# scenarios/VAE-2

Measured on AMD Instinct MI355X. Metric: training frames/sec on 128x256 8-frame Cityscapes clips, 1/2/4/8 MI355X, higher is better.
Workload: dtype fp32; 1 GPU; VAE2 ELBO step (encz + encoder + 2 decoders fwd/bwd + Adam), HRNet-W18-small-v2, 128x256, 8 clips/GPU x 9 frames (CLIP_LENGTH=3); yaml=vae-2_amd/experiments/vae2_w18_small_v2_128x256.yaml, global_batch=8, frames_per_clip=9, parallelism=dp1, sync_bn=False, launch=hip_graph, mfma_operands=fp32

## Files before the change

### vae-2_amd/csrc/common.h

```cpp
#pragma once

#include <hip/hip_runtime.h>
#include <stdint.h>
#include <string>
#include <stdio.h>

#include "../../include/vae2_hip.h"

namespace vae2 {

constexpr int kSyncMaxRanks = 8;

void set_error(const std::string& msg);
int fail(const char* fn, const std::string& msg);
int check_launch(const char* fn);

void note_kernel(const void* host_fn);
#define VAE2_LAUNCH(K, ...)                                         \
  do {                                                              \
    ::vae2::note_kernel(reinterpret_cast<const void*>(K));          \
    hipLaunchKernelGGL(K, __VA_ARGS__);                             \
  } while (0)

#define VAE2_REQUIRE(cond, fn, msg)          \
// ... 123 lines not shown
struct FastDiv {
  uint32_t d, m, s;
  FastDiv() : d(1), m(0), s(0) {}
  explicit FastDiv(uint32_t div) : d(div) {
    for (s = 0; s < 32; ++s)
      if ((1u << s) >= d) break;
    uint64_t one = 1;
    m = (uint32_t)(((one << 32) * ((one << s) - d)) / d + 1);
  }
  __device__ __forceinline__ uint32_t div(uint32_t n) const {
    return (__umulhi(n, m) + n) >> s;
  }
};

struct Lerp {
  int i0, i1;
  float l0, l1;
};

__device__ __forceinline__ Lerp lerp_index(int dst, int in_size, float scale) {
  float src = scale * ((float)dst + 0.5f) - 0.5f;
  if (src < 0.f) src = 0.f;
  int i0 = (int)src;
  if (i0 > in_size - 1) i0 = in_size - 1;
  int ip = (i0 < in_size - 1) ? 1 : 0;
  Lerp l;
  l.i0 = i0;
  l.i1 = i0 + ip;
  l.l1 = src - (float)i0;
  l.l0 = 1.f - l.l1;
  return l;
}

__device__ __forceinline__ float lerp_weight(int o, int in_size, float scale, int i) {
  Lerp l = lerp_index(o, in_size, scale);
  float w = 0.f;
  if (l.i0 == i) w += l.l0;
  if (l.i1 == i) w += l.l1;
  return w;
}

__device__ constexpr float hat_w(int d, int f) {
  return 1.f - (float)(2 * d + 1 - f < 0 ? f - 1 - 2 * d : 2 * d + 1 - f) / (float)(2 * f);
}

int adj3_fuse_launch(const float* dy, const vae2_act* dyd, int n, float* const* dxs,
                     const vae2_act* dxds, const float* betas, hipStream_t st);
extern int g_relu_dual_q;

int64_t wgrad3n_splits(const vae2_act* xd, const vae2_act* dyd);
int wgrad3n_launch(const float* x, const vae2_act* xd, const float* dy, const vae2_act* dyd,
                   float* part, const float* isave, int irelu, uint32_t x_bytes,
                   uint32_t dy_bytes, hipStream_t s);

extern int g_dconv_stream, g_dconv_stream_wpc, g_dconv_stream_bl, g_dconv_stream_spb,
    g_wgrad_narrow_tps, g_bn_blocks, g_bn_apply_res, g_fuse_quad;
bool dconv3s_shape(const vae2_act* ad, const vae2_act* yd);
int64_t dconv3s_rows(const vae2_act* ad, const vae2_act* yd);
int dconv3s_launch(const float* a, const vae2_act* ad, const float* wp, uint32_t w_bytes,
                   const float* bias, float* y, const vae2_act* yd, float beta, float* stats,
                   bool flip, const float* isave, int irelu, const float* bx, int bx_ps,
                   int brelu, const float* bsave, uint32_t bx_bytes, uint32_t a_bytes,
                   hipStream_t s);

int bias_grad_from_partials(const float* partials, int64_t rows, int64_t c,
                            float* dbias, int accumulate, void* stream);

inline unsigned ew_blocks(int64_t n, int threads = 256, int64_t cap = 65536) {
  int64_t b = ceil_div(n, threads);
  if (b > cap) b = cap;
  if (b < 1) b = 1;
  return (unsigned)b;
}

}
```

### vae-2_amd/csrc/conv.hip

```cpp
#include <mutex>
#include <vector>

#include "common.h"

#ifndef VAE2_ABLATE
#define VAE2_ABLATE 0
#endif

#ifndef VAE2_CONV_PART
#define VAE2_CONV_PART -1
#endif
#define VAE2_PART(n) (VAE2_CONV_PART < 0 || VAE2_CONV_PART == (n))

namespace vae2 {


static inline int round_up(int a, int b) { return (a + b - 1) / b * b; }

#if VAE2_PART(0)
__global__ void pack_weight_kernel(const float* __restrict__ w, int cout, int cin, int kk,
                                   int mode, int ld, float* __restrict__ out) {
  const int rows = mode == 0 ? (cout + 63) / 64 * 64 : (cin + 63) / 64 * 64;
  const int cols4 = mode == 0 ? (cin + 3) / 4 * 4 : (cout + 3) / 4 * 4;
  const int total = rows * kk * cols4;
// ... 575 lines not shown
template <int TM, int TN>
__global__ __launch_bounds__(256) void gemm1x1_kernel(Gemm1 p) {
  constexpr int BN = 16 * TN;
  extern __shared__ __attribute__((aligned(16))) float bsh[];
  __shared__ float red[4][2][BN];
  const int lane = threadIdx.x & 63, wave = threadIdx.x >> 6;
  const int g = lane >> 4, r = lane & 15;
  const int n0 = blockIdx.y * BN;
  const int nch = (p.a_c4 + 15) >> 4;
  const int KL = nch * 16 + 4;
  {
    const __amdgpu_buffer_rsrc_t wr = make_rsrc(p.w, p.w_bytes);
    const int q4 = nch * 4;
    for (int i = threadIdx.x; i < BN * q4; i += 256) {
      const int nn = i / q4, q = i - nn * q4;
      const bool ok = 4 * q < p.a_c4;
      const f4 v = load4(wr, ok ? (uint32_t)((n0 + nn) * p.a_c4 + 4 * q) * 4u : kOOB);
      *reinterpret_cast<f4*>(&bsh[nn * KL + 4 * q]) = v;
    }
  }
  const __amdgpu_buffer_rsrc_t ar = make_rsrc(p.a, p.a_bytes);
  const int ntiles = (p.M + 16 * TM - 1) / (16 * TM);
  const int t0 = blockIdx.x * 4 + wave, tstep = gridDim.x * 4;
  const int iters = t0 < ntiles ? (ntiles - t0 + tstep - 1) / tstep : 0;
  const int S = iters * nch;
  const bool cpad = (p.a_c & 3) != 0;
  float bv[TN];
#pragma unroll
  for (int j = 0; j < TN; ++j) {
    const int n = n0 + j * 16 + r;
    bv[j] = (p.bias && n < p.n) ? p.bias[n] : 0.f;
  }
  f4 acc[TM][TN];
#pragma unroll
  for (int i = 0; i < TM; ++i)
#pragma unroll
    for (int j = 0; j < TN; ++j) acc[i][j] = f4{0.f, 0.f, 0.f, 0.f};
  float csum[TN], csq[TN];
#pragma unroll
  for (int j = 0; j < TN; ++j) { csum[j] = 0.f; csq[j] = 0.f; }
  const bool bnp = p.bx != nullptr;
  float pmn[TN], pis[TN], psc[TN], psh[TN];
#pragma unroll
  for (int j = 0; j < TN; ++j) {
    const int n = n0 + j * 16 + r < p.n ? n0 + j * 16 + r : p.n - 1;
    pmn[j] = bnp ? p.bsave[n] : 0.f;
    pis[j] = bnp ? p.bsave[p.n + n] : 0.f;
    psc[j] = bnp ? p.bsave[2 * p.n + n] : 0.f;
    psh[j] = bnp ? p.bsave[3 * p.n + n] : 0.f;
  }
  const __amdgpu_buffer_rsrc_t bxr = make_rsrc(p.bx, bnp ? p.bx_bytes : 0u);
  __syncthreads();

  auto load = [&](f4* fa, int st) {
    const int it = st / nch, c = st - it * nch;
    const int t = t0 + it * tstep;
    const int q = 16 * c + 4 * g;
#pragma unroll
    for (int i = 0; i < TM; ++i) {
      const int m = t * 16 * TM + i * 16 + r;
      const bool ok = st < S && m < p.M && q < p.a_c4;
      fa[i] = load4(ar, ok ? (uint32_t)(m * p.a_ps + q) * 4u : kOOB);
    }
  };
  auto mma = [&](f4* fa, int st) {
    const int it = st / nch, c = st - it * nch;
    if (cpad && c == nch - 1) {
      const int q = 16 * c + 4 * g;
#pragma unroll
      for (int i = 0; i < TM; ++i) {
        fa[i][1] = q + 1 < p.a_c ? fa[i][1] : 0.f;
        fa[i][2] = q + 2 < p.a_c ? fa[i][2] : 0.f;
        fa[i][3] = q + 3 < p.a_c ? fa[i][3] : 0.f;
      }
    }
    f4 fb[TN];
#pragma unroll
    for (int j = 0; j < TN; ++j)
      fb[j] = *reinterpret_cast<const f4*>(&bsh[(j * 16 + r) * KL + 16 * c + 4 * g]);
#pragma unroll
    for (int s2 = 0; s2 < 4; ++s2)
#pragma unroll
      for (int i = 0; i < TM; ++i)
#pragma unroll
        for (int j = 0; j < TN; ++j)
          acc[i][j] = __builtin_amdgcn_mfma_f32_16x16x4f32(fa[i][s2], fb[j][s2], acc[i][j], 0, 0, 0);
  };
  auto epi = [&](int st) {
    const int it = st / nch, c = st - it * nch;
    if (c != nch - 1) return;
    const int t = t0 + it * tstep;
    const int k = r & 3, qc = 4 * (r >> 2);
#pragma unroll
    for (int i = 0; i < TM; ++i) {
      const int mb = t * 16 * TM + i * 16 + 4 * g;
      if (p.stats && bnp) {
        float xv[4][TN];
#pragma unroll
        for (int e = 0; e < 4; ++e)
#pragma unroll
          for (int j = 0; j < TN; ++j) {
            const int n = n0 + j * 16 + r;
            xv[e][j] = load1(bxr, mb + e < p.M && n < p.n
                                      ? (uint32_t)((mb + e) * p.bx_ps + n) * 4u : kOOB);
          }
#pragma unroll
        for (int e = 0; e < 4; ++e) {
#pragma unroll
          for (int j = 0; j < TN; ++j) {
            const bool ok = mb + e < p.M && n0 + j * 16 + r < p.n;
            const float v = acc[i][j][e];
            const float x = xv[e][j];
            const float gv = (p.brelu && !(__builtin_fmaf(x, psc[j], psh[j]) > 0.f)) ? 0.f : v;
            csum[j] += ok ? gv : 0.f;
            csq[j] += ok ? gv * (x - pmn[j]) * pis[j] : 0.f;
          }
        }
      } else if (p.stats) {
#pragma unroll
        for (int e = 0; e < 4; ++e) {
#pragma unroll
          for (int j = 0; j < TN; ++j) {
            if (mb + e < p.M && n0 + j * 16 + r < p.n) {
              const float v = acc[i][j][e] + bv[j];
              csum[j] += v;
              csq[j] += v * v;
            }
          }
        }
      }
      const int m = mb + k;
      float* yrow = p.y + (int64_t)m * p.y_ps;
      f4 yold[TN];
      if (p.beta != 0.f) {
#pragma unroll
        for (int j = 0; j < TN; ++j) {
          const int n = n0 + j * 16 + qc;
          yold[j] = (p.vec && m < p.M && n + 3 < p.n) ? *reinterpret_cast<const f4*>(yrow + n)
                                                      : f4{0.f, 0.f, 0.f, 0.f};
        }
      }
#pragma unroll
      for (int j = 0; j < TN; ++j) {
        f4 v = acc[i][j];
        acc[i][j] = f4{0.f, 0.f, 0.f, 0.f};
        quad_transpose(v, k);
        const int n = n0 + j * 16 + qc;
        if (m >= p.M || n >= p.n) continue;
        if (p.bias) {
#pragma unroll
          for (int q = 0; q < 4; ++q) v[q] += n + q < p.n ? p.bias[n + q] : 0.f;
        }
        if (p.vec && n + 3 < p.n) {
          if (p.beta != 0.f) v += p.beta * yold[j];
          *reinterpret_cast<f4*>(yrow + n) = v;
        } else {
#pragma unroll
          for (int q = 0; q < 4; ++q)
            if (n + q < p.n) yrow[n + q] = p.beta != 0.f ? v[q] + p.beta * yrow[n + q] : v[q];
        }
      }
    }
  };
  if (S > 0) {
    f4 fa0[TM], fa1[TM];
    load(fa0, 0);
    load(fa1, 1);
    for (int st = 0; st < S; st += 2) {
      mma(fa0, st);
      load(fa0, st + 2);
      epi(st);
      if (st + 1 < S) {
        mma(fa1, st + 1);
        load(fa1, st + 3);
        epi(st + 1);
      }
    }
  }
  if (p.stats) {
#pragma unroll
    for (int j = 0; j < TN; ++j) {
      csum[j] += __shfl_xor(csum[j], 16, 64);
      csum[j] += __shfl_xor(csum[j], 32, 64);
      csq[j] += __shfl_xor(csq[j], 16, 64);
      csq[j] += __shfl_xor(csq[j], 32, 64);
    }
    if (g == 0) {
#pragma unroll
      for (int j = 0; j < TN; ++j) {
        red[wave][0][j * 16 + r] = csum[j];
        red[wave][1][j * 16 + r] = csq[j];
      }
    }
    __syncthreads();
    const int rows = gridDim.x;
    for (int c = threadIdx.x; c < BN; c += 256) {
      if (n0 + c >= p.n) continue;
      p.stats[blockIdx.x * p.n + n0 + c] = red[0][0][c] + red[1][0][c] + red[2][0][c] + red[3][0][c];
      p.stats[(rows + blockIdx.x) * p.n + n0 + c] =
          red[0][1][c] + red[1][1][c] + red[2][1][c] + red[3][1][c];
    }
  }
}

struct DConv {
  const float* a;
  int a_ps, a_c, a_c4, img_h, img_w;
  int tiles_h, tiles_w;
  int cs4;
  const float* w;
  uint32_t a_bytes, w_bytes;
  int n;
  const float* bias;
  float* y;
  int y_ps;
  float beta;
  float* stats;
  const float* isave;
  int irelu;
  const float* bx;
  int bx_ps, brelu;
  const float* bsave;
  uint32_t bx_bytes;
  int vec_out;
};

constexpr int kDcBW = 32;
constexpr int kDcMaxCs4 = 8;
// ... 1858 lines not shown
  }
  if (key == 1) {
    const int prev = g_wgrad_cols;
    g_wgrad_cols = value ? 1 : 0;
    return prev;
  }
  if (key == 2) {
    const int prev = g_dconv_nw8;
    g_dconv_nw8 = value ? 1 : 0;
    return prev;
  }
  if (key == 3) {
    const int prev = g_wgrad_nw8;
    g_wgrad_nw8 = value ? 1 : 0;
    return prev;
  }
  if (key == 4) {
    if (value < 3 || value > 8) return -1;
    const int prev = g_gemm1_tn;
    g_gemm1_tn = value;
    return prev;
  }
  if (key == 5) {
    const int prev = g_gemm1_tm;
    g_gemm1_tm = value == 1 ? 1 : 2;
    return prev;
  }
  if (key == 6) {
    if (value < 0 || value > 2) return -1;
    const int prev = g_igemm_nr;
    g_igemm_nr = value;
    return prev;
  }
  if (key == 8) {
    const int prev = g_bn_v2;
    g_bn_v2 = value ? 1 : 0;
    return prev;
  }
  if (key == 7) {
    if (value < 0 || value > 3) return -1;
    const int prev = g_wgrad_narrow;
    g_wgrad_narrow = value;
    return prev;
  }
  if (key == 9) {
    const int prev = g_dconv_stream;
    g_dconv_stream = value >= 0 && value <= 3 ? value : 3;
    return prev;
  }
  if (key == 18) {
    if (value < 256 || value > 8192) return -1;
    const int prev = g_wgrad_wgs;
    g_wgrad_wgs = value;
    return prev;
  }
  if (key == 21) {
    const int prev = g_fuse_quad;
    g_fuse_quad = value ? 1 : 0;
    return prev;
  }
  if (key == 20) {
    if (value < 0 || value > 65536) return -1;
    const int prev = g_bn_apply_res;
    g_bn_apply_res = value;
    return prev;
  }
  if (key == 19) {
    if (value < 256 || value > 8192) return -1;
    const int prev = g_bn_blocks;
    g_bn_blocks = value;
    return prev;
  }
  if (key == 16) {
    if (value < 1 || value > 2) return -1;
    const int prev = g_wgrad_narrow_tps;
    g_wgrad_narrow_tps = value;
    return prev;
  }
  if (key == 17) {
    if (value < 1 || value > 2) return -1;
    const int prev = g_dconv_stream_spb;
    g_dconv_stream_spb = value;
    return prev;
  }
  if (key == 15) {
    if (value < 0 || value > 2) return -1;
    const int prev = g_dconv_ksp;
    g_dconv_ksp = value;
    return prev;
  }
  if (key == 14) {
    const int prev = g_dconv_split72;
    g_dconv_split72 = value ? 1 : 0;
    return prev;
  }
  if (key == 13) {
    const int prev = g_dconv_n16;
    g_dconv_n16 = value ? 1 : 0;
    return prev;
  }
  if (key == 12) {
    const int prev = g_igemm_tab;
    g_igemm_tab = value ? 1 : 0;
    return prev;
  }
  if (key == 11) {
// ... 409 lines not shown
                                          J.beta, stream);
      if (rc) return rc;
      continue;
    }
    const DTile d = pick_dtile(ad, od, false);
    const uint32_t wb = (uint32_t)((fwd ? vae2_conv2d_packed_size(od->c, ad->c, J.k, 0)
                                        : vae2_conv2d_packed_size(ad->c, od->c, J.k, 1)) * 4);
    int k = 0;
    while (k < nb && !(b[k].tm == d.tm && b[k].tn == d.tn && b[k].flip == (fwd ? 0 : 1))) ++k;
    if (k == nb) {
      VAE2_REQUIRE(nb < 8, fn, "too many tile shapes");
      b[nb] = Bucket{};
      b[nb].tm = d.tm; b[nb].tn = d.tn; b[nb].flip = fwd ? 0 : 1;
      ++nb;
    }
    Bucket& B = b[k];
    if (B.cnt == kDcGroup) {
      int rc = flush(B);
      if (rc) return rc;
    }
    const int tiles = (int)(ad->n * d.tiles_h * d.tiles_w);
    B.g.p[B.cnt] = make_dconv(d, J.x, ad, J.wp, wb, fwd ? J.bias : nullptr, J.y, od, J.beta,
                              fwd ? J.stats : nullptr);
    B.g.start[B.cnt] = B.tot;
    B.g.tiles[B.cnt] = tiles;
    B.outs[B.cnt] = J.y;
    B.tot += tiles * d.nblk;
    const size_t sh = dconv_shm(d);
    if (sh > B.shm) B.shm = sh;
    ++B.cnt;
  }
  for (int k = 0; k < nb; ++k) {
    int rc = flush(b[k]);
    if (rc) return rc;
  }
  return 0;
}

#endif

#if VAE2_PART(3)
int64_t vae2_conv2d_bwd_weight_ws_size(const vae2_act* xd, const vae2_act* dyd, int k) {
  if (!act_ok(xd) || !act_ok(dyd)) return 0;
  int ncol4 = k * k * round_up((int)xd->c, 4);
  WTile t = pick_wtile(act_pixels(dyd), (int)dyd->c, ncol4);
  int64_t part = (int64_t)t.splits * dyd->c * ncol4;
  if ((k == 3 || k == 1) && xd->h == dyd->h && xd->w == dyd->w) {
    W3Tile t3 = pick_w3tile(xd, dyd, k);
    const int64_t part3 = (int64_t)t3.splits * dyd->c * ncol4;
    if (part3 > part) part = part3;
    const int64_t partn = wgrad3n_splits(xd, dyd) * dyd->c * ncol4;
    if (partn > part) part = partn;
  }
  int64_t bias_part = 2 * vae2_bn_partial_rows(dyd) * dyd->c;
  return part + bias_part + 4;
}

static int bwd_weight_impl(const float* x, const vae2_act* xd, const float* dy,
                           const vae2_act* dyd, float* dw, int64_t dw_ld, float* dbias,
                           int k, int stride, int pad, int accumulate, float* ws,
                           int64_t ws_size, void* stream, const float* isave, int irelu,
                           const char* fn) {
  VAE2_REQUIRE(xd && dw_ld >= xd->c * k * k, fn, "bad dW row stride");
  VAE2_REQUIRE(x && dy && dw && ws, fn, "null pointer");
  VAE2_REQUIRE(conv_shapes_ok(xd, dyd, k, stride, pad), fn, "inconsistent conv shapes");
  VAE2_REQUIRE(fits32(xd) && fits32(dyd), fn, "tensor too large for 32-bit indexing");
  VAE2_REQUIRE(ws_size >= vae2_conv2d_bwd_weight_ws_size(xd, dyd, k), fn, "workspace too small");
  hipStream_t s = as_stream(stream);
  const int cin4 = round_up((int)xd->c, 4);
  const int ncol4 = k * k * cin4;
  int splits = 0;
  const bool direct = g_conv_algo != 1 && wgrad3_shape_ok(xd, dyd, k, stride, pad) &&
                      vec_ok(x, (int)xd->ps) && vec_ok(dy, (int)dyd->ps);
  VAE2_REQUIRE(direct || !isave, fn,
               "input BatchNorm needs the direct 3x3 weight-gradient kernel (vae2_conv2d_bnin_ok)");
  if (direct && k == 3) {
    splits = wgrad3n_launch(x, xd, dy, dyd, ws, isave, irelu, act_bytes(xd), act_bytes(dyd), s);
    if (splits < 0) return check_launch(fn);
  }
  if (direct && !splits) {
    W3Tile t3 = pick_w3tile(xd, dyd, k);
    WGrad3 q{};
    q.x = x; q.x_ps = (int)xd->ps; q.cin = (int)xd->c; q.cin4 = cin4;
    q.h = (int)xd->h; q.w = (int)xd->w;
    q.dy = dy; q.dy_ps = (int)dyd->ps; q.cout = (int)dyd->c;
    q.tiles_h = t3.tiles_h; q.tiles_w = t3.tiles_w; q.ntiles = t3.ntiles;
    q.tiles_per_split = t3.tps;
    q.csw = t3.csw; q.n_ci_slabs = t3.n_ci_slabs;
    q.x_bytes = act_bytes(xd); q.dy_bytes = act_bytes(dyd);
    q.part = ws;
    q.isave = isave;
    q.irelu = irelu ? 1 : 0;
    dim3 grid((unsigned)t3.splits, (unsigned)(t3.n_ci_slabs * t3.n_co_slabs));
    const size_t shm = wgrad3_lds(t3);
    if (t3.bh == 8) wgrad3_launch<8>(q, t3, grid, shm, s);
    else wgrad3_launch<4>(q, t3, grid, shm, s);
    int rc = check_launch(fn);
    if (rc) return rc;
    splits = t3.splits;
  }
  WTile t = pick_wtile(act_pixels(dyd), (int)dyd->c, ncol4);
  if (splits) goto reduce;
  {
  WGrad p{};
  p.x = x; p.x_ps = (int)xd->ps; p.cin = (int)xd->c; p.cin4 = cin4;
  p.x_h = (int)xd->h; p.x_w = (int)xd->w;
  p.dy = dy; p.dy_ps = (int)dyd->ps; p.cout = (int)dyd->c;
  p.o_n = (int)dyd->n; p.o_h = (int)dyd->h; p.o_w = (int)dyd->w;
  p.k = k; p.stride = stride; p.pad = pad;
  p.P = (int)act_pixels(dyd);
  p.px_split = t.px_split;
  p.part = ws;
  p.x_bytes = act_bytes(xd);
  p.dy_bytes = act_bytes(dyd);
  p.ohw_div = FastDiv((uint32_t)(dyd->h * dyd->w));
  p.ow_div = FastDiv((uint32_t)dyd->w);
  p.cin4_div = FastDiv((uint32_t)cin4);
  dim3 grid(t.gx, t.gy, (unsigned)t.splits);
  const bool v4 = g_vec_out && vec_ok(x, (int)xd->ps) && vec_ok(dy, (int)dyd->ps);
  switch (t.tm) {
    case 1: launch_wgrad_tn<1>(p, t.tn, grid, s, v4); break;
    case 2: launch_wgrad_tn<2>(p, t.tn, grid, s, v4); break;
    case 3: launch_wgrad_tn<3>(p, t.tn, grid, s, v4); break;
    default: launch_wgrad_tn<4>(p, t.tn, grid, s, v4); break;
  }
  int rc = check_launch(fn);
  if (rc) return rc;
  splits = t.splits;
  }
reduce:
  int64_t slab = dyd->c * (int64_t)ncol4;
  int rc = 0;
  if (g_wr_defer) {
    WRJob j{ws, dw, dw_ld, splits, (int)dyd->c, (int)xd->c, cin4, k, accumulate, 0};
    std::lock_guard<std::mutex> lk(g_wr_mu);
    g_wr_queue.push_back(WRQueued{j, s});
  } else {
    VAE2_LAUNCH(wgrad_reduce_kernel, dim3((unsigned)ceil_div(slab, 32)), dim3(256), 0, s,
                (const float*)ws, splits, (int)dyd->c, (int)xd->c, cin4, k, dw, dw_ld,
                accumulate);
    rc = check_launch(fn);
    if (rc) return rc;
  }
  if (dbias) {
    const int64_t part_max = vae2_conv2d_bwd_weight_ws_size(xd, dyd, k) - 4 -
                             2 * vae2_bn_partial_rows(dyd) * dyd->c;
    float* bp = ws + part_max;
    rc = vae2_bn_stats(dy, dyd, bp, stream);
    if (rc) return rc;
    rc = bias_grad_from_partials(bp, vae2_bn_partial_rows(dyd), dyd->c, dbias, accumulate,
                                 stream);
    if (rc) return rc;
// ... 34 lines not shown
```

### vae-2_amd/csrc/wgrad_narrow.hip

```cpp
#include "common.h"

namespace vae2 {

extern int g_bf16, g_wgrad_narrow;
int g_wgrad_narrow_tps = 2;

constexpr int kTH = 4;
constexpr int kTW = 32;
constexpr int kLW = kTW + 2;
constexpr int kNPX = kTH * kTW;

struct WGN {
  const float* x;
  int x_ps, cin, cin4, h, w;
  const float* dy;
  int dy_ps, cout;
  int tiles_h, tiles_w, ntiles, tps;
  int n_ci_slabs;
  FastDiv per_img_div, tiles_w_div;
  uint32_t x_bytes, dy_bytes;
  float* part;
  const float* isave;
  int irelu;
};
// ... 335 lines not shown

bool plan(const vae2_act* xd, const vae2_act* dyd, Plan& pl) {
  if (g_bf16 || !g_wgrad_narrow || !pick(xd, dyd, pl.c)) return false;
  pl.tiles_h = (int)ceil_div(dyd->h, kTH);
  pl.tiles_w = (int)ceil_div(dyd->w, kTW);
  pl.ntiles = (int)(dyd->n * pl.tiles_h * pl.tiles_w);
  const int gy = pl.c.ci_slabs * pl.c.co_slabs;
  int64_t want = (int64_t)256 * resident_per_cu(pl.c) / gy;
  if (want < 1) want = 1;
  pl.tps = (int)ceil_div(pl.ntiles, want);
  if (pl.tps < g_wgrad_narrow_tps) pl.tps = g_wgrad_narrow_tps;
  pl.splits = (int)ceil_div(pl.ntiles, pl.tps);
  return true;
}

}

int64_t wgrad3n_splits(const vae2_act* xd, const vae2_act* dyd) {
  Plan pl;
  return plan(xd, dyd, pl) ? pl.splits : 0;
}

int wgrad3n_launch(const float* x, const vae2_act* xd, const float* dy, const vae2_act* dyd,
                   float* part, const float* isave, int irelu, uint32_t x_bytes,
                   uint32_t dy_bytes, hipStream_t s) {
  Plan pl;
  if (!plan(xd, dyd, pl)) return 0;
  WGN p{};
  p.x = x; p.x_ps = (int)xd->ps; p.cin = (int)xd->c; p.cin4 = (int)((xd->c + 3) / 4 * 4);
  p.h = (int)xd->h; p.w = (int)xd->w;
  p.dy = dy; p.dy_ps = (int)dyd->ps; p.cout = (int)dyd->c;
  p.tiles_h = pl.tiles_h; p.tiles_w = pl.tiles_w; p.ntiles = pl.ntiles; p.tps = pl.tps;
  p.n_ci_slabs = pl.c.ci_slabs;
  p.per_img_div = FastDiv((uint32_t)(pl.tiles_h * pl.tiles_w));
  p.tiles_w_div = FastDiv((uint32_t)pl.tiles_w);
  p.x_bytes = x_bytes; p.dy_bytes = dy_bytes;
  p.part = part;
  p.isave = isave; p.irelu = irelu ? 1 : 0;
  dim3 grid((unsigned)pl.splits, (unsigned)(pl.c.ci_slabs * pl.c.co_slabs));
  const size_t shm = lds_bytes(pl.c);
  if (pl.c.cq == 5) {
    if (pl.c.nw == 8) VAE2_LAUNCH((wgrad3n_kernel<5, 1, 2, 4, false, 8>), grid, dim3(512), shm, s, p);
    else if (pl.c.pf) VAE2_LAUNCH((wgrad3n_kernel<5, 1, 2, 2, true>), grid, dim3(256), shm, s, p);
    else VAE2_LAUNCH((wgrad3n_kernel<5, 1, 2, 2, false>), grid, dim3(256), shm, s, p);
  } else {
    if (pl.c.nw == 8) VAE2_LAUNCH((wgrad3n_kernel<9, 2, 4, 2, false, 8>), grid, dim3(512), shm, s, p);
    else if (pl.c.pf) VAE2_LAUNCH((wgrad3n_kernel<9, 2, 4, 1, true>), grid, dim3(256), shm, s, p);
    else VAE2_LAUNCH((wgrad3n_kernel<9, 2, 4, 1, false>), grid, dim3(256), shm, s, p);
  }
  const hipError_t e = hipGetLastError();
  return e == hipSuccess ? pl.splits : -(int)e;
}

}
```

### vae-2_amd/csrc/build.py

```python
import concurrent.futures as cf
import os
import shutil
import subprocess
import sys

HERE = os.path.dirname(os.path.abspath(__file__))
PKG = os.path.join(os.path.dirname(HERE), "vae2")
TAG = os.environ.get("VAE2_BUILD_TAG", "")
DEFS = os.environ.get("VAE2_DEFS", "").split()
OUT = os.path.join(PKG, f"libvae2_hip_{TAG}.so" if TAG else "libvae2_hip.so")
BUILD = os.path.join(HERE, f"build_{TAG}" if TAG else "build")
SOURCES = ["conv.hip", "bn.hip", "resample.hip", "elbo.hip", "heads.hip", "clips.hip",
           "metrics.hip", "wgrad_narrow.hip", "syncbn.hip", "dconv_stream.hip",
           "ssim_loss.hip"]
HEADERS = ["common.h", os.path.join("..", "..", "include", "vae2_hip.h")]
ARCH = os.environ.get("VAE2_OFFLOAD_ARCH", "gfx950")
FLAGS = ["-O3", "-std=c++17", "-fPIC", f"--offload-arch={ARCH}", "-Wall",
         "-Wno-unused-function", "-munsafe-fp-atomics"]
EXTRA = {"conv.hip": ["-fno-slp-vectorize"], "dconv_stream.hip": ["-fno-slp-vectorize"]}
PARTS = {"conv.hip": 4}


def _units():
    out = []
    for src in SOURCES:
        n = PARTS.get(src, 0)
        base = os.path.splitext(src)[0]
        if n:
            out += [(src, f"{base}_p{i}.o", [f"-DVAE2_CONV_PART={i}"]) for i in range(n)]
        else:
            out.append((src, base + ".o", []))
    return out


def hipcc():
    for cand in (os.environ.get("HIPCC"), "/opt/rocm/bin/hipcc", shutil.which("hipcc")):
        if cand and os.path.exists(cand):
            return cand
    raise RuntimeError("hipcc not found (set HIPCC)")


def _newer(target, deps):
    if not os.path.exists(target):
        return True
    t = os.path.getmtime(target)
    return any(os.path.getmtime(d) > t for d in deps)


def _compile(unit):
    src, oname, defs = unit
    obj = os.path.join(BUILD, oname)
    deps = [os.path.join(HERE, src)] + [os.path.join(HERE, h) for h in HEADERS]
    if not _newer(obj, deps):
        return obj, None
    cmd = [hipcc()] + FLAGS + EXTRA.get(src, []) + defs + DEFS + ["-c", os.path.join(HERE, src), "-o", obj]
    r = subprocess.run(cmd, capture_output=True, text=True)
    if r.returncode != 0:
        return obj, f"$ {' '.join(cmd)}\n{r.stdout}\n{r.stderr}"
    return obj, None


def build(verbose=True, force=False):
    os.makedirs(BUILD, exist_ok=True)
    if force:
        for f in os.listdir(BUILD):
            os.remove(os.path.join(BUILD, f))
    units = _units()
# ... 19 lines not shown
```

Measured before the change: 930.7 frames/s.

## Add specialized MFMA weight-gradient kernel for stride-2 3x3 convolutions

Adds a dedicated weight-gradient kernel for 3x3 stride-2 pad-1 convolutions that stages an input halo tile in LDS with even and odd columns de-interleaved, so the strided taps read contiguously. It accumulates with fp32 MFMA and writes split-K partials that go through the existing reduction path. The kernel is enabled by default for the HRNet channel combinations it knows and replaces the generic im2col-style wgrad path for downsampling convs. It also enlarges the workspace sizing and picks the number of splits from occupancy.

```diff
diff --git a/vae-2_amd/csrc/common.h b/vae-2_amd/csrc/common.h
--- a/vae-2_amd/csrc/common.h
+++ b/vae-2_amd/csrc/common.h
@@ -199,6 +199,10 @@
 int wgrad3n_launch(const float* x, const vae2_act* xd, const float* dy, const vae2_act* dyd,
                    float* part, const float* isave, int irelu, uint32_t x_bytes,
                    uint32_t dy_bytes, hipStream_t s);
+extern int g_wgrad_s2;
+int64_t wgrad3s2_splits(const vae2_act* xd, const vae2_act* dyd);
+int wgrad3s2_launch(const float* x, const vae2_act* xd, const float* dy, const vae2_act* dyd,
+                    float* part, uint32_t x_bytes, uint32_t dy_bytes, hipStream_t s);
 
 extern int g_dconv_stream, g_dconv_stream_wpc, g_dconv_stream_bl, g_dconv_stream_spb,
     g_wgrad_narrow_tps, g_bn_blocks, g_bn_apply_res, g_fuse_quad;
diff --git a/vae-2_amd/csrc/conv.hip b/vae-2_amd/csrc/conv.hip
--- a/vae-2_amd/csrc/conv.hip
+++ b/vae-2_amd/csrc/conv.hip
@@ -2737,6 +2737,12 @@
     if (value < 256 || value > 8192) return -1;
     const int prev = g_wgrad_wgs;
     g_wgrad_wgs = value;
+    return prev;
+  }
+  if (key == 22) {
+    if (value < 0 || value > 2) return -1;
+    const int prev = g_wgrad_s2;
+    g_wgrad_s2 = value;
     return prev;
   }
   if (key == 21) {
@@ -3252,6 +3258,10 @@
     const int64_t partn = wgrad3n_splits(xd, dyd) * dyd->c * ncol4;
     if (partn > part) part = partn;
   }
+  if (k == 3 && dyd->h == (xd->h + 1) / 2 && dyd->w == (xd->w + 1) / 2) {
+    const int64_t parts2 = wgrad3s2_splits(xd, dyd) * dyd->c * ncol4;
+    if (parts2 > part) part = parts2;
+  }
   int64_t bias_part = 2 * vae2_bn_partial_rows(dyd) * dyd->c;
   return part + bias_part + 4;
 }
@@ -3298,6 +3308,11 @@
     int rc = check_launch(fn);
     if (rc) return rc;
     splits = t3.splits;
+  }
+  if (!splits && g_wgrad_s2 && g_conv_algo != 1 && k == 3 && stride == 2 && pad == 1 &&
+      vec_ok(x, (int)xd->ps) && vec_ok(dy, (int)dyd->ps)) {
+    splits = wgrad3s2_launch(x, xd, dy, dyd, ws, act_bytes(xd), act_bytes(dyd), s);
+    if (splits < 0) return check_launch(fn);
   }
   WTile t = pick_wtile(act_pixels(dyd), (int)dyd->c, ncol4);
   if (splits) goto reduce;
diff --git a/vae-2_amd/csrc/wgrad_narrow.hip b/vae-2_amd/csrc/wgrad_narrow.hip
--- a/vae-2_amd/csrc/wgrad_narrow.hip
+++ b/vae-2_amd/csrc/wgrad_narrow.hip
@@ -411,4 +411,372 @@
   return e == hipSuccess ? pl.splits : -(int)e;
 }
 
-}
+int g_wgrad_s2 = 1;
+
+constexpr int kTH2 = 4;
+constexpr int kTW2 = 16;
+constexpr int kLH2 = 2 * kTH2 + 1;
+constexpr int kLW2 = 2 * kTW2 + 1;
+constexpr int kNPX2 = kTH2 * kTW2;
+
+struct WGS2 {
+  const float* x;
+  int x_ps, cin, cin4, h, w;
+  const float* dy;
+  int dy_ps, cout, oh, ow;
+  int tiles_h, tiles_w, ntiles, tps;
+  int n_ci_slabs;
+  FastDiv per_img_div, tiles_w_div;
+  uint32_t x_bytes, dy_bytes;
+  float* part;
+};
+
+template <int CQ, int TM, int NR, int WPIX, int NW>
+__global__ __launch_bounds__(64 * NW) void wgrad3s2_kernel(WGS2 p) {
+  constexpr int CSW = 4 * CQ;
+  constexpr int CO = 16 * TM + NR;
+  constexpr int COQ = (CO + 3) / 4;
+  constexpr int DP = 4 * COQ;
+  constexpr int XP = CSW;
+  constexpr int LPX = kLH2 * kLW2;
+  constexpr int RS = kLW2 * XP + ((CSW - kLW2 * XP) % 16 + 16) % 16;
+  constexpr int PO = (kTW2 + 1) * XP;
+  constexpr int G = (3 * CSW + 15) / 16;
+  constexpr int WCOL = NW / WPIX;
+  constexpr int NT = 64 * NW;
+  constexpr int GW = (G + WCOL - 1) / WCOL;
+  static_assert(NR <= 4 && (NR == 0 || COQ == 4 * TM + 1), "one remainder quad");
+  static_assert(WCOL * WPIX == NW && WPIX <= kTH2, "waves per tile");
+  extern __shared__ __attribute__((aligned(16))) float sm[];
+  float* xs = sm;
+  float* ds = sm + kLH2 * RS;
+
+  const int lane = threadIdx.x & 63, wave = threadIdx.x >> 6;
+  const int g = lane >> 4, r = lane & 15;
+  const int wc = wave % WCOL, wp = wave / WCOL;
+  const int cis = blockIdx.y % p.n_ci_slabs, cos = blockIdx.y / p.n_ci_slabs;
+  const int c0 = cis * CSW, co0 = cos * CO;
+  const __amdgpu_buffer_rsrc_t xr = make_rsrc(p.x, p.x_bytes);
+  const __amdgpu_buffer_rsrc_t dr = make_rsrc(p.dy, p.dy_bytes);
+
+  int xoff[GW];
+  bool colok[GW];
+#pragma unroll
+  for (int j = 0; j < GW; ++j) {
+    const int n = (wc * GW + j) * 16 + r;
+    const int nc = n < 3 * CSW ? n : 3 * CSW - 1;
+    const int dh = nc / CSW, ci = nc - dh * CSW;
+    colok[j] = wc * GW + j < G && n < 3 * CSW && c0 + ci < p.cin;
+    xoff[j] = dh * RS + ci;
+  }
+
+  f4 acc[TM][GW][3];
+#pragma unroll
+  for (int i = 0; i < TM; ++i)
+#pragma unroll
+    for (int j = 0; j < GW; ++j)
+#pragma unroll
+      for (int d = 0; d < 3; ++d) acc[i][j][d] = f4{0.f, 0.f, 0.f, 0.f};
+  float racc[GW][3][NR > 0 ? NR : 1];
+#pragma unroll
+  for (int j = 0; j < GW; ++j)
+#pragma unroll
+    for (int d = 0; d < 3; ++d)
+#pragma unroll
+      for (int q = 0; q < NR; ++q) racc[j][d][q] = 0.f;
+
+  const int per_img = p.tiles_h * p.tiles_w;
+  const int tb = blockIdx.x * p.tps;
+  const int te = tb + p.tps < p.ntiles ? tb + p.tps : p.ntiles;
+  constexpr int XPU = NT / CQ, DPU = NT / COQ;
+  constexpr int NXI = (LPX + XPU - 1) / XPU, NDI = (kNPX2 + DPU - 1) / DPU;
+  const int xq = threadIdx.x % CQ, xb = threadIdx.x / CQ;
+  const int dq = threadIdx.x % COQ, db = threadIdx.x / COQ;
+  const bool xact = xb < XPU, dact = db < DPU;
+  const int xc = c0 + 4 * xq;
+  const bool xcok = xc < p.cin4;
+  const bool dcok = co0 + 4 * dq < p.cout;
+
+  for (int tile = tb; tile < te; ++tile) {
+    const int img = (int)p.per_img_div.div((uint32_t)tile);
+    const int trem = tile - img * per_img;
+    const int th = (int)p.tiles_w_div.div((uint32_t)trem);
+    const int oh0 = th * kTH2, ow0 = (trem - th * p.tiles_w) * kTW2;
+    f4 px[NXI], pd[NDI];
+#pragma unroll
+    for (int u = 0; u < NXI; ++u) {
+      const int hp = xb + u * XPU;
+      const int lr = hp / kLW2, q = hp - lr * kLW2;
+      const int lc = q <= kTW2 ? 2 * q : 2 * (q - kTW2) - 1;
+      const int ih = 2 * oh0 - 1 + lr, iw = 2 * ow0 - 1 + lc;
+      const bool ok = xact && hp < LPX && xcok && (unsigned)ih < (unsigned)p.h &&
+                      (unsigned)iw < (unsigned)p.w;
+      px[u] = load4(xr, ok ? (uint32_t)(((img * p.h + ih) * p.w + iw) * p.x_ps + xc) * 4u : kOOB);
+    }
+#pragma unroll
+    for (int u = 0; u < NDI; ++u) {
+      const int pp = db + u * DPU;
+      const int oh = oh0 + pp / kTW2, ow = ow0 + (pp & (kTW2 - 1));
+      const bool ok = dact && pp < kNPX2 && dcok && oh < p.oh && ow < p.ow;
+      pd[u] = load4(dr, ok ? (uint32_t)(((img * p.oh + oh) * p.ow + ow) * p.dy_ps + co0 + 4 * dq) * 4u : kOOB);
+    }
+    __syncthreads();
+#pragma unroll
+    for (int u = 0; u < NXI; ++u) {
+      const int hp = xb + u * XPU;
+      if (!xact || hp >= LPX) break;
+      f4 v = px[u];
+#pragma unroll
+      for (int k = 0; k < 4; ++k) v[k] = xc + k < p.cin ? v[k] : 0.f;
+      const int lr = hp / kLW2, q = hp - lr * kLW2;
+      *reinterpret_cast<f4*>(&xs[lr * RS + q * XP + 4 * xq]) = v;
+    }
+#pragma unroll
+    for (int u = 0; u < NDI; ++u) {
+      const int pp = db + u * DPU;
+      if (!dact || pp >= kNPX2) break;
+      f4 v = pd[u];
+#pragma unroll
+      for (int k = 0; k < 4; ++k) v[k] = (co0 + 4 * dq + k < p.cout && 4 * dq + k < CO) ? v[k] : 0.f;
+      *reinterpret_cast<f4*>(&ds[pp * DP + 4 * dq]) = v;
+    }
+    __syncthreads();
+#pragma unroll 1
+    for (int orow = wp; orow < kTH2; orow += WPIX) {
+      const int dpx = orow * kTW2 + 4 * g;
+      float a[TM][4];
+#pragma unroll
+      for (int i = 0; i < TM; ++i)
+#pragma unroll
+        for (int s = 0; s < 4; ++s) a[i][s] = ds[(dpx + s) * DP + 16 * i + r];
+      f4 rq[4];
+      if constexpr (NR > 0) {
+#pragma unroll
+        for (int s = 0; s < 4; ++s) rq[s] = *reinterpret_cast<const f4*>(&ds[(dpx + s) * DP + 16 * TM]);
+      }
+      const int xrow = 2 * orow * RS + 4 * g * XP;
+#pragma unroll
+      for (int j = 0; j < GW; ++j) {
+        float xv[9];
+#pragma unroll
+        for (int t = 0; t < 9; ++t) xv[t] = xs[xrow + xoff[j] + (t & 1) * PO + (t >> 1) * XP];
+#pragma unroll
+        for (int d = 0; d < 3; ++d) {
+#pragma unroll
+          for (int s = 0; s < 4; ++s)
+#pragma unroll
+            for (int i = 0; i < TM; ++i)
+              acc[i][j][d] = __builtin_amdgcn_mfma_f32_16x16x4f32(a[i][s], xv[2 * s + d], acc[i][j][d], 0, 0, 0);
+          if constexpr (NR > 0) {
+#pragma unroll
+            for (int q = 0; q < NR; ++q)
+#pragma unroll
+              for (int s = 0; s < 4; ++s) racc[j][d][q] = __builtin_fmaf(rq[s][q], xv[2 * s + d], racc[j][d][q]);
+          }
+        }
+      }
+    }
+  }
+
+#pragma unroll
+  for (int j = 0; j < GW; ++j)
+#pragma unroll
+    for (int d = 0; d < 3; ++d)
+#pragma unroll
+      for (int q = 0; q < NR; ++q) {
+        float v = racc[j][d][q];
+        v += __shfl_xor(v, 16, 64);
+        v += __shfl_xor(v, 32, 64);
+        racc[j][d][q] = v;
+      }
+  const int ncol4 = 9 * p.cin4;
+  const uint32_t slab = (uint32_t)(p.cout * ncol4);
+  const __amdgpu_buffer_rsrc_t orr = make_rsrc(p.part + (int64_t)blockIdx.x * slab, slab * 4u);
+  int colb[GW];
+#pragma unroll
+  for (int j = 0; j < GW; ++j) {
+    const int n = (wc * GW + j) * 16 + r;
+    const int dh = n / CSW, ci = n - dh * CSW;
+    colb[j] = colok[j] ? dh * 3 * p.cin4 + c0 + ci : -1;
+  }
+  if constexpr (WPIX > 1) {
+    constexpr int NV = TM * GW * 3 * 4 + GW * 3 * NR;
+    __syncthreads();
+    float* red = sm;
+    if (wp > 0) {
+      float* o = red + ((wp - 1) * WCOL + wc) * NV * 64 + lane;
+      int k = 0;
+#pragma unroll
+      for (int i = 0; i < TM; ++i)
+#pragma unroll
+        for (int j = 0; j < GW; ++j)
+#pragma unroll
+          for (int d = 0; d < 3; ++d)
+#pragma unroll
+            for (int e = 0; e < 4; ++e) o[64 * k++] = acc[i][j][d][e];
+#pragma unroll
+      for (int j = 0; j < GW; ++j)
+#pragma unroll
+        for (int d = 0; d < 3; ++d)
+#pragma unroll
+          for (int q = 0; q < NR; ++q) o[64 * k++] = racc[j][d][q];
+    }
+    __syncthreads();
+    if (wp > 0) return;
+#pragma unroll 1
+    for (int w = 1; w < WPIX; ++w) {
+      const float* o = red + ((w - 1) * WCOL + wc) * NV * 64 + lane;
+      int k = 0;
+#pragma unroll
+      for (int i = 0; i < TM; ++i)
+#pragma unroll
+        for (int j = 0; j < GW; ++j)
+#pragma unroll
+          for (int d = 0; d < 3; ++d)
+#pragma unroll
+            for (int e = 0; e < 4; ++e) acc[i][j][d][e] += o[64 * k++];
+#pragma unroll
+      for (int j = 0; j < GW; ++j)
+#pragma unroll
+        for (int d = 0; d < 3; ++d)
+#pragma unroll
+          for (int q = 0; q < NR; ++q) racc[j][d][q] += o[64 * k++];
+    }
+  }
+#pragma unroll
+  for (int j = 0; j < GW; ++j)
+#pragma unroll
+    for (int d = 0; d < 3; ++d) {
+      const uint32_t col = (uint32_t)(colb[j] + d * p.cin4);
+#pragma unroll
+      for (int i = 0; i < TM; ++i)
+#pragma unroll
+        for (int e = 0; e < 4; ++e) {
+          const int co = co0 + 16 * i + 4 * g + e;
+          store1(orr, colb[j] >= 0 && co < p.cout ? ((uint32_t)(co * ncol4) + col) * 4u : kOOB,
+                 acc[i][j][d][e]);
+        }
+#pragma unroll
+      for (int q = 0; q < NR; ++q) {
+        const int co = co0 + 16 * TM + q;
+        store1(orr, g == 0 && colb[j] >= 0 && co < p.cout ? ((uint32_t)(co * ncol4) + col) * 4u : kOOB,
+               racc[j][d][q]);
+      }
+    }
+}
+
+namespace {
+
+struct Cfg2 {
+  int cq, tm, nr, wpix, ci_slabs, co_slabs, nw;
+};
+
+bool pick2(const vae2_act* xd, const vae2_act* dyd, Cfg2& c) {
+  const int64_t ci = xd->c, co = dyd->c;
+  const bool wide = co == 36 || co == 72 || co == 144;
+  const bool w8 = g_wgrad_narrow == 3;
+  if (ci == 18 && co == 18) c = Cfg2{5, 1, 2, w8 ? 4 : 2, 1, 1, w8 ? 8 : 4};
+  else if (ci == 18 && wide) c = Cfg2{5, 2, 4, 2, 1, (int)(co / 36), w8 ? 8 : 4};
+  else if (ci == 36 && wide) c = Cfg2{9, 2, 4, w8 ? 2 : 1, 1, (int)(co / 36), w8 ? 8 : 4};
+  else if (ci == 72 && co == 144) c = Cfg2{9, 2, 4, w8 ? 2 : 1, 2, 4, w8 ? 8 : 4};
+  else return false;
+  return true;
+}
+
+size_t lds_bytes2(const Cfg2& c) {
+  const int CO = 16 * c.tm + c.nr, DP = 4 * ((CO + 3) / 4);
+  const int csw = 4 * c.cq, rs = kLW2 * csw + ((csw - kLW2 * csw) % 16 + 16) % 16;
+  const size_t stage = ((size_t)kLH2 * rs + (size_t)kNPX2 * DP) * sizeof(float);
+  const int G = (3 * csw + 15) / 16, wcol = c.nw / c.wpix, gw = (G + wcol - 1) / wcol;
+  const size_t nv = (size_t)c.tm * gw * 12 + (size_t)gw * 3 * c.nr;
+  const size_t red = (size_t)(c.wpix - 1) * wcol * nv * 64 * sizeof(float);
+  return stage > red ? stage : red;
+}
+
+template <typename F>
+void with_kernel2(const Cfg2& c, F&& f) {
+  const bool w8 = c.nw == 8;
+  if (c.cq == 5 && c.tm == 1) {
+    if (w8) f(wgrad3s2_kernel<5, 1, 2, 4, 8>, 0);
+    else f(wgrad3s2_kernel<5, 1, 2, 2, 4>, 1);
+  } else if (c.cq == 5) {
+    if (w8) f(wgrad3s2_kernel<5, 2, 4, 2, 8>, 2);
+    else f(wgrad3s2_kernel<5, 2, 4, 2, 4>, 3);
+  } else {
+    if (w8) f(wgrad3s2_kernel<9, 2, 4, 2, 8>, 4);
+    else f(wgrad3s2_kernel<9, 2, 4, 1, 4>, 5);
+  }
+}
+
+int resident_per_cu2(const Cfg2& c) {
+  static int cache[6] = {0, 0, 0, 0, 0, 0};
+  int n = 0;
+  with_kernel2(c, [&](auto kernel, int k) {
+    if (!cache[k]) {
+      if (hipOccupancyMaxActiveBlocksPerMultiprocessor(&cache[k], reinterpret_cast<const void*>(kernel),
+                                                       64 * c.nw, lds_bytes2(c)) != hipSuccess ||
+          cache[k] < 1) {
+        (void)hipGetLastError();
+        cache[k] = 1;
+      }
+    }
+    n = cache[k];
+  });
+  return n;
+}
+
+struct Plan2 {
+  Cfg2 c;
+  int tiles_h, tiles_w, ntiles, tps, splits;
+};
+
+bool plan2(const vae2_act* xd, const vae2_act* dyd, Plan2& pl) {
+  if (g_bf16 || !g_wgrad_s2 || !pick2(xd, dyd, pl.c)) return false;
+  if (dyd->h != (xd->h + 1) / 2 || dyd->w != (xd->w + 1) / 2 || dyd->n != xd->n) return false;
+  pl.tiles_h = (int)ceil_div(dyd->h, kTH2);
+  pl.tiles_w = (int)ceil_div(dyd->w, kTW2);
+  pl.ntiles = (int)(dyd->n * pl.tiles_h * pl.tiles_w);
+  if (pl.c.tm == 1 && pl.ntiles >= 256 && pl.ntiles < 512) return false;
+  const int gy = pl.c.ci_slabs * pl.c.co_slabs;
+  int64_t want = (int64_t)256 * resident_per_cu2(pl.c) / gy;
+  if (want < 1) want = 1;
+  pl.tps = (int)ceil_div(pl.ntiles, want);
+  int min_tps = g_wgrad_narrow_tps;
+  if (g_wgrad_s2 == 1 && ceil_div(pl.ntiles, min_tps) * gy < 256) min_tps = 1;
+  if (pl.tps < min_tps) pl.tps = min_tps;
+  pl.splits = (int)ceil_div(pl.ntiles, pl.tps);
+  return true;
+}
+
+}
+
+int64_t wgrad3s2_splits(const vae2_act* xd, const vae2_act* dyd) {
+  Plan2 pl;
+  return plan2(xd, dyd, pl) ? pl.splits : 0;
+}
+
+int wgrad3s2_launch(const float* x, const vae2_act* xd, const float* dy, const vae2_act* dyd,
+                    float* part, uint32_t x_bytes, uint32_t dy_bytes, hipStream_t s) {
+  Plan2 pl;
+  if (!plan2(xd, dyd, pl)) return 0;
+  WGS2 p{};
+  p.x = x; p.x_ps = (int)xd->ps; p.cin = (int)xd->c; p.cin4 = (int)((xd->c + 3) / 4 * 4);
+  p.h = (int)xd->h; p.w = (int)xd->w;
+  p.dy = dy; p.dy_ps = (int)dyd->ps; p.cout = (int)dyd->c;
+  p.oh = (int)dyd->h; p.ow = (int)dyd->w;
+  p.tiles_h = pl.tiles_h; p.tiles_w = pl.tiles_w; p.ntiles = pl.ntiles; p.tps = pl.tps;
+  p.n_ci_slabs = pl.c.ci_slabs;
+  p.per_img_div = FastDiv((uint32_t)(pl.tiles_h * pl.tiles_w));
+  p.tiles_w_div = FastDiv((uint32_t)pl.tiles_w);
+  p.x_bytes = x_bytes; p.dy_bytes = dy_bytes;
+  p.part = part;
+  const dim3 grid((unsigned)pl.splits, (unsigned)(pl.c.ci_slabs * pl.c.co_slabs));
+  const size_t shm = lds_bytes2(pl.c);
+  with_kernel2(pl.c, [&](auto kernel, int) {
+    VAE2_LAUNCH(kernel, grid, dim3(64 * pl.c.nw), shm, s, p);
+  });
+  const hipError_t e = hipGetLastError();
+  return e == hipSuccess ? pl.splits : -(int)e;
+}
+
+}
```

New measurement: 937.4 frames/s, median of 6. Within noise of the previous version (+0.7%).

## Add dedicated MFMA 1x1 weight-gradient kernel and simplify conv loader indexing

Applied to the files above, without the earlier changes.

Adds a new split-K HIP kernel for 1x1 stride-1 convolution weight gradients on large pixel counts. It tiles cout x cin across waves, splits pixels across workgroups, reduces partial sums across waves through LDS and writes per-split partials into the workspace. This is meant to replace the generic weight-gradient path for 1x1 convs. Separately, a conv kernel's pipelined loop now keeps incremental row and chunk counters instead of dividing the step index each iteration. The risks are more workspace use and more partial-sum traffic to reduce afterwards.

```diff
diff --git a/vae-2_amd/csrc/build.py b/vae-2_amd/csrc/build.py
--- a/vae-2_amd/csrc/build.py
+++ b/vae-2_amd/csrc/build.py
@@ -12,7 +12,7 @@
 BUILD = os.path.join(HERE, f"build_{TAG}" if TAG else "build")
 SOURCES = ["conv.hip", "bn.hip", "resample.hip", "elbo.hip", "heads.hip", "clips.hip",
            "metrics.hip", "wgrad_narrow.hip", "syncbn.hip", "dconv_stream.hip",
-           "ssim_loss.hip"]
+           "ssim_loss.hip", "wgrad_1x1.hip"]
 HEADERS = ["common.h", os.path.join("..", "..", "include", "vae2_hip.h")]
 ARCH = os.environ.get("VAE2_OFFLOAD_ARCH", "gfx950")
 FLAGS = ["-O3", "-std=c++17", "-fPIC", f"--offload-arch={ARCH}", "-Wall",
diff --git a/vae-2_amd/csrc/common.h b/vae-2_amd/csrc/common.h
--- a/vae-2_amd/csrc/common.h
+++ b/vae-2_amd/csrc/common.h
@@ -200,6 +200,12 @@
                    float* part, const float* isave, int irelu, uint32_t x_bytes,
                    uint32_t dy_bytes, hipStream_t s);
 
+extern int g_wgrad_1x1;
+int64_t wgrad1x1_splits(const vae2_act* xd, const vae2_act* dyd, int k, int stride, int pad);
+int wgrad1x1_launch(const float* x, const vae2_act* xd, const float* dy, const vae2_act* dyd,
+                    int k, int stride, int pad, float* part, uint32_t x_bytes,
+                    uint32_t dy_bytes, hipStream_t s);
+
 extern int g_dconv_stream, g_dconv_stream_wpc, g_dconv_stream_bl, g_dconv_stream_spb,
     g_wgrad_narrow_tps, g_bn_blocks, g_bn_apply_res, g_fuse_quad;
 bool dconv3s_shape(const vae2_act* ad, const vae2_act* yd);
diff --git a/vae-2_amd/csrc/conv.hip b/vae-2_amd/csrc/conv.hip
--- a/vae-2_amd/csrc/conv.hip
+++ b/vae-2_amd/csrc/conv.hip
@@ -651,21 +651,36 @@
   const __amdgpu_buffer_rsrc_t bxr = make_rsrc(p.bx, bnp ? p.bx_bytes : 0u);
   __syncthreads();
 
-  auto load = [&](f4* fa, int st) {
-    const int it = st / nch, c = st - it * nch;
-    const int t = t0 + it * tstep;
-    const int q = 16 * c + 4 * g;
+  int lt = t0, lc = 0, lleft = iters;
+  uint32_t lrow[TM];
+  auto lrows = [&]() {
 #pragma unroll
     for (int i = 0; i < TM; ++i) {
-      const int m = t * 16 * TM + i * 16 + r;
-      const bool ok = st < S && m < p.M && q < p.a_c4;
-      fa[i] = load4(ar, ok ? (uint32_t)(m * p.a_ps + q) * 4u : kOOB);
+      const int m = lt * 16 * TM + i * 16 + r;
+      const bool ok = lleft > 0 && m < p.M;
+      lrow[i] = ok ? (uint32_t)(m * p.a_ps) * 4u : kOOB;
     }
   };
-  auto mma = [&](f4* fa, int st) {
-    const int it = st / nch, c = st - it * nch;
-    if (cpad && c == nch - 1) {
-      const int q = 16 * c + 4 * g;
+  lrows();
+  auto load = [&](f4* fa) {
+    const int q = 16 * lc + 4 * g;
+    const bool qok = q < p.a_c4;
+#pragma unroll
+    for (int i = 0; i < TM; ++i) fa[i] = load4(ar, qok ? lrow[i] + (uint32_t)q * 4u : kOOB);
+    if (++lc == nch) {
+      lc = 0;
+      lt += tstep;
+      --lleft;
+      lrows();
+    }
+  };
+  int mt = t0, mc = 0;
+  int boff[TN];
+#pragma unroll
+  for (int j = 0; j < TN; ++j) boff[j] = (j * 16 + r) * KL + 4 * g;
+  auto mma = [&](f4* fa) {
+    if (cpad && mc == nch - 1) {
+      const int q = 16 * mc + 4 * g;
 #pragma unroll
       for (int i = 0; i < TM; ++i) {
         fa[i][1] = q + 1 < p.a_c ? fa[i][1] : 0.f;
@@ -676,7 +691,7 @@
     f4 fb[TN];
 #pragma unroll
     for (int j = 0; j < TN; ++j)
-      fb[j] = *reinterpret_cast<const f4*>(&bsh[(j * 16 + r) * KL + 16 * c + 4 * g]);
+      fb[j] = *reinterpret_cast<const f4*>(&bsh[boff[j] + 16 * mc]);
 #pragma unroll
     for (int s2 = 0; s2 < 4; ++s2)
 #pragma unroll
@@ -685,10 +700,8 @@
         for (int j = 0; j < TN; ++j)
           acc[i][j] = __builtin_amdgcn_mfma_f32_16x16x4f32(fa[i][s2], fb[j][s2], acc[i][j], 0, 0, 0);
   };
-  auto epi = [&](int st) {
-    const int it = st / nch, c = st - it * nch;
-    if (c != nch - 1) return;
-    const int t = t0 + it * tstep;
+  auto epi = [&]() {
+    const int t = mt;
     const int k = r & 3, qc = 4 * (r >> 2);
 #pragma unroll
     for (int i = 0; i < TM; ++i) {
@@ -761,18 +774,27 @@
       }
     }
   };
+  auto next = [&]() {
+    if (mc == nch - 1) {
+      epi();
+      mc = 0;
+      mt += tstep;
+    } else {
+      ++mc;
+    }
+  };
   if (S > 0) {
     f4 fa0[TM], fa1[TM];
-    load(fa0, 0);
-    load(fa1, 1);
+    load(fa0);
+    load(fa1);
     for (int st = 0; st < S; st += 2) {
-      mma(fa0, st);
-      load(fa0, st + 2);
-      epi(st);
+      mma(fa0);
+      load(fa0);
+      next();
       if (st + 1 < S) {
-        mma(fa1, st + 1);
-        load(fa1, st + 3);
-        epi(st + 1);
+        mma(fa1);
+        load(fa1);
+        next();
       }
     }
   }
@@ -2737,6 +2759,12 @@
     if (value < 256 || value > 8192) return -1;
     const int prev = g_wgrad_wgs;
     g_wgrad_wgs = value;
+    return prev;
+  }
+  if (key == 22) {
+    if (value < 0 || value > 1) return -1;
+    const int prev = g_wgrad_1x1;
+    g_wgrad_1x1 = value;
     return prev;
   }
   if (key == 21) {
@@ -3252,6 +3280,8 @@
     const int64_t partn = wgrad3n_splits(xd, dyd) * dyd->c * ncol4;
     if (partn > part) part = partn;
   }
+  const int64_t part1 = wgrad1x1_splits(xd, dyd, k, 1, 0) * dyd->c * ncol4;
+  if (part1 > part) part = part1;
   int64_t bias_part = 2 * vae2_bn_partial_rows(dyd) * dyd->c;
   return part + bias_part + 4;
 }
@@ -3277,6 +3307,12 @@
   if (direct && k == 3) {
     splits = wgrad3n_launch(x, xd, dy, dyd, ws, isave, irelu, act_bytes(xd), act_bytes(dyd), s);
     if (splits < 0) return check_launch(fn);
+  }
+  if (!direct && !isave && vec_ok(x, (int)xd->ps) && vec_ok(dy, (int)dyd->ps)) {
+    splits = wgrad1x1_launch(x, xd, dy, dyd, k, stride, pad, ws, act_bytes(xd), act_bytes(dyd), s);
+    if (splits < 0)
+      return fail(fn, std::string("1x1 weight-gradient launch: ") +
+                          hipGetErrorString((hipError_t)-splits));
   }
   if (direct && !splits) {
     W3Tile t3 = pick_w3tile(xd, dyd, k);
diff --git a/vae-2_amd/csrc/wgrad_1x1.hip b/vae-2_amd/csrc/wgrad_1x1.hip
--- /dev/null
+++ b/vae-2_amd/csrc/wgrad_1x1.hip
@@ -0,0 +1,218 @@
+#include "common.h"
+
+namespace vae2 {
+
+extern int g_bf16;
+int g_wgrad_1x1 = 1;
+
+static constexpr int64_t kMinPixels = 32768;
+static constexpr int kWgs = 256;
+static constexpr int kMinPxWg = 128;
+
+struct WG1 {
+  const float* x;
+  const float* dy;
+  float* part;
+  int x_ps, dy_ps, cin4, cout;
+  int P, px_wg;
+  int wc_sh, nrc_sh, wp_n;
+  uint32_t x_bytes, dy_bytes;
+};
+
+template <int TM, int TN>
+__global__ __launch_bounds__(512) void wgrad1x1_kernel(WG1 p) {
+  extern __shared__ __attribute__((aligned(16))) float wred[];
+  const int lane = threadIdx.x & 63;
+  const int wave = __builtin_amdgcn_readfirstlane((int)(threadIdx.x >> 6));
+  const int g = lane >> 4, r = lane & 15, kq = r & 3, q4 = r & 12;
+  const int wpi = wave >> p.nrc_sh, wrc = wave & ((1 << p.nrc_sh) - 1);
+  const int wr = wrc >> p.wc_sh, wc = wrc & ((1 << p.wc_sh) - 1);
+  const int pbeg = blockIdx.x * p.px_wg;
+  const int pend = min(pbeg + p.px_wg, p.P);
+  const __amdgpu_buffer_rsrc_t xr =
+      make_rsrc(p.x, min(p.x_bytes, (uint32_t)pend * (uint32_t)p.x_ps * 4u));
+  const __amdgpu_buffer_rsrc_t dr =
+      make_rsrc(p.dy, min(p.dy_bytes, (uint32_t)pend * (uint32_t)p.dy_ps * 4u));
+
+  uint32_t dcol[TM], xcol[TN];
+#pragma unroll
+  for (int i = 0; i < TM; ++i) {
+    const int co = (wr * TM + i) * 16 + q4;
+    dcol[i] = co < p.cout ? (uint32_t)co * 4u : kOOB;
+  }
+#pragma unroll
+  for (int j = 0; j < TN; ++j) {
+    const int ci = (wc * TN + j) * 16 + q4;
+    xcol[j] = ci < p.cin4 ? (uint32_t)ci * 4u : kOOB;
+  }
+  f4 acc[TM][TN];
+#pragma unroll
+  for (int i = 0; i < TM; ++i)
+#pragma unroll
+    for (int j = 0; j < TN; ++j) acc[i][j] = f4{0.f, 0.f, 0.f, 0.f};
+
+  const int px0 = pbeg + 16 * wpi + 4 * g + kq;
+  uint32_t drow = (uint32_t)px0 * (uint32_t)p.dy_ps * 4u;
+  uint32_t xrow = (uint32_t)px0 * (uint32_t)p.x_ps * 4u;
+  const uint32_t dstep = 64u * (uint32_t)p.wp_n * (uint32_t)p.dy_ps;
+  const uint32_t xstep = 64u * (uint32_t)p.wp_n * (uint32_t)p.x_ps;
+  auto load = [&](f4* fa, f4* fb) {
+#pragma unroll
+    for (int i = 0; i < TM; ++i) fa[i] = load4(dr, drow + dcol[i]);
+#pragma unroll
+    for (int j = 0; j < TN; ++j) fb[j] = load4(xr, xrow + xcol[j]);
+    drow += dstep;
+    xrow += xstep;
+  };
+  auto step = [&](f4* fa, f4* fb) {
+    f4 ta[TM], tb[TN];
+#pragma unroll
+    for (int i = 0; i < TM; ++i) {
+      ta[i] = fa[i];
+      quad_transpose(ta[i], kq);
+    }
+#pragma unroll
+    for (int j = 0; j < TN; ++j) {
+      tb[j] = fb[j];
+      quad_transpose(tb[j], kq);
+    }
+    load(fa, fb);
+#pragma unroll
+    for (int s = 0; s < 4; ++s)
+#pragma unroll
+      for (int i = 0; i < TM; ++i)
+#pragma unroll
+        for (int j = 0; j < TN; ++j)
+          acc[i][j] = __builtin_amdgcn_mfma_f32_16x16x4f32(ta[i][s], tb[j][s], acc[i][j], 0, 0, 0);
+  };
+  {
+    f4 a0[TM], b0[TN], a1[TM], b1[TN];
+    const int stride = 16 * p.wp_n;
+    load(a0, b0);
+    load(a1, b1);
+    for (int pc = pbeg + 16 * wpi; pc < pend; pc += 2 * stride) {
+      step(a0, b0);
+      step(a1, b1);
+    }
+  }
+
+  constexpr int NV = TM * TN * 4;
+  float* mine = wred + (size_t)wrc * NV * 64 + lane;
+  for (int w = 1; w < p.wp_n; ++w) {
+    if (wpi == w) {
+#pragma unroll
+      for (int i = 0; i < TM; ++i)
+#pragma unroll
+        for (int j = 0; j < TN; ++j)
+#pragma unroll
+          for (int e = 0; e < 4; ++e) mine[((i * TN + j) * 4 + e) * 64] = acc[i][j][e];
+    }
+    __syncthreads();
+    if (wpi == 0) {
+#pragma unroll
+      for (int i = 0; i < TM; ++i)
+#pragma unroll
+        for (int j = 0; j < TN; ++j)
+#pragma unroll
+          for (int e = 0; e < 4; ++e) acc[i][j][e] += mine[((i * TN + j) * 4 + e) * 64];
+    }
+    __syncthreads();
+  }
+  if (wpi != 0) return;
+
+  float* out = p.part + (int64_t)blockIdx.x * p.cout * p.cin4;
+#pragma unroll
+  for (int i = 0; i < TM; ++i)
+#pragma unroll
+    for (int e = 0; e < 4; ++e) {
+      const int co = (wr * TM + i) * 16 + g * 4 + e;
+      if (co >= p.cout) continue;
+#pragma unroll
+      for (int j = 0; j < TN; ++j) {
+        const int col = (wc * TN + j) * 16 + r;
+        if (col < p.cin4) out[(int64_t)co * p.cin4 + col] = acc[i][j][e];
+      }
+    }
+}
+
+namespace {
+
+struct Inst {
+  int tm, tn;
+};
+constexpr Inst kInst[] = {{4, 4}, {5, 2}, {5, 3}};
+constexpr int kNInst = sizeof(kInst) / sizeof(kInst[0]);
+
+struct Plan {
+  int inst, wr_sh, wc_sh, wp, px_wg, splits;
+  size_t lds;
+};
+
+bool plan(const vae2_act* xd, const vae2_act* dyd, int k, int stride, int pad, Plan& pl) {
+  if (g_bf16 || !g_wgrad_1x1) return false;
+  if (k != 1 || stride != 1 || pad != 0) return false;
+  if (xd->ps % 4 || dyd->ps % 4) return false;
+  const int64_t P = act_pixels(dyd);
+  if (P < kMinPixels) return false;
+  const int rt = (int)ceil_div(dyd->c, 16), ct = (int)ceil_div(ceil_div(xd->c, 4) * 4, 16);
+  int best = -1;
+  for (int wr_sh = 0; wr_sh <= 3; ++wr_sh)
+    for (int wc_sh = 0; wr_sh + wc_sh <= 3; ++wc_sh) {
+      const int wr = 1 << wr_sh, wc = 1 << wc_sh, wp = 8 / (wr * wc);
+      const int tm = (int)ceil_div(rt, wr), tn = (int)ceil_div(ct, wc);
+      for (int n = 0; n < kNInst; ++n) {
+        const Inst& I = kInst[n];
+        if (I.tm < tm || I.tn < tn) continue;
+        const size_t lds = wp > 1 ? (size_t)wr * wc * I.tm * I.tn * 4 * 64 * sizeof(float) : 0;
+        if (lds > 65536) continue;
+        const int cost = wr * wc * (I.tm * I.tn * 64 + I.tm + I.tn);
+        if (best < 0 || cost < best) {
+          best = cost;
+          pl.inst = n; pl.wr_sh = wr_sh; pl.wc_sh = wc_sh; pl.wp = wp; pl.lds = lds;
+        }
+      }
+    }
+  if (best < 0) return false;
+  {
+    const Inst& I = kInst[pl.inst];
+    const int padded = I.tm * I.tn << (pl.wr_sh + pl.wc_sh);
+    if (3 * rt * ct < 2 * padded) return false;
+  }
+  int64_t px = ceil_div(ceil_div(P, kWgs), 16) * 16;
+  if (px < kMinPxWg) px = kMinPxWg;
+  pl.px_wg = (int)px;
+  pl.splits = (int)ceil_div(P, px);
+  return true;
+}
+
+}
+
+int64_t wgrad1x1_splits(const vae2_act* xd, const vae2_act* dyd, int k, int stride, int pad) {
+  Plan pl;
+  return plan(xd, dyd, k, stride, pad, pl) ? pl.splits : 0;
+}
+
+int wgrad1x1_launch(const float* x, const vae2_act* xd, const float* dy, const vae2_act* dyd,
+                    int k, int stride, int pad, float* part, uint32_t x_bytes,
+                    uint32_t dy_bytes, hipStream_t s) {
+  Plan pl;
+  if (!plan(xd, dyd, k, stride, pad, pl)) return 0;
+  if (((uintptr_t)x | (uintptr_t)dy) & 15) return 0;
+  WG1 p{};
+  p.x = x; p.dy = dy; p.part = part;
+  p.x_ps = (int)xd->ps; p.dy_ps = (int)dyd->ps;
+  p.cin4 = (int)(ceil_div(xd->c, 4) * 4); p.cout = (int)dyd->c;
+  p.P = (int)act_pixels(dyd); p.px_wg = pl.px_wg;
+  p.wc_sh = pl.wc_sh; p.nrc_sh = pl.wr_sh + pl.wc_sh; p.wp_n = pl.wp;
+  p.x_bytes = x_bytes; p.dy_bytes = dy_bytes;
+  const dim3 grid((unsigned)pl.splits), block(512);
+  switch (pl.inst) {
+    case 0: VAE2_LAUNCH((wgrad1x1_kernel<4, 4>), grid, block, pl.lds, s, p); break;
+    case 1: VAE2_LAUNCH((wgrad1x1_kernel<5, 2>), grid, block, pl.lds, s, p); break;
+    default: VAE2_LAUNCH((wgrad1x1_kernel<5, 3>), grid, block, pl.lds, s, p); break;
+  }
+  const hipError_t e = hipGetLastError();
+  return e == hipSuccess ? pl.splits : -(int)e;
+}
+
+}
```

New measurement: 930.2 frames/s before, 940.1 frames/s after, median of 6. +1.1%, better.
